# KdaiP/StableTTS

Measured on NVIDIA B200. Metric: mel-frames/sec through CFM DiT estimator (ODE solve, all evaluations), higher is better.
Workload: dtype f32 (split-bf16x3 tensor-core operands; FFN convs fp16 activations x fp16 hi/lo weights, 2 passes; fp32 accumulate)

## Files before the change

stabletts_b200/csrc/gemm_epilogue.cuh:

```cuda
#pragma once
#include "common.cuh"
#include <cstdlib>
#include "tc_ptx.cuh"

namespace st {

enum : int { EM_PLAIN = 0, EM_SILU = 1, EM_GELU = 2, EM_ROPE = 3, EM_LN = 4, EM_RESID = 5 };

struct EpiMaps { CUtensorMap o_f32, o_hi, o_lo, o2_f32, u_hi, u_lo, resid; };

struct TcParams {
    int n_src, Cs0, Cs1, taps, N, a_bmod, BB, T;
    int m_tiles_per_b, n_tiles, total_tiles;
    int flags, B, film_H, c_clamp, resid_clamp, rope_H, tap_outer;
    long film_bstride, gate_bstride;
    const float *bias, *mask, *film, *gate, *resid, *rope_cs;
    int mode;
    int has_f32, has_split;
    int out16, u16;
    int ln_mask_out, has_film2;
    const float *ln_shift, *ln_scale, *film2;
    long ada_bstride, film2_bstride;
    int ksplit, split_bb;
    long long* dbg;
// ... 12 lines not shown
    p.n_src = g.n_src; p.Cs0 = g.Cs[0]; p.Cs1 = g.Cs[1]; p.taps = g.taps; p.N = g.N; p.a_bmod = g.a_bmod; p.BB = g.BB; p.T = g.T;
    p.flags = g.flags; p.B = g.B; p.film_H = g.film_H; p.c_clamp = g.c_clamp; p.resid_clamp = g.resid_clamp; p.rope_H = g.rope_H;
    p.film_bstride = g.film_bstride; p.gate_bstride = g.gate_bstride;
    p.bias = g.bias; p.mask = g.mask; p.film = g.film; p.gate = g.gate; p.resid = g.resid; p.rope_cs = g.rope_cs;
    p.mode = epilogue_mode(g);
    p.has_f32 = g.out_f32 != nullptr; p.has_split = g.out_hi != nullptr;
    p.out16 = g.out16; p.u16 = g.u16;
    p.ln_mask_out = g.ln_mask_out; p.has_film2 = g.film2 != nullptr;
    p.ln_shift = g.ln_shift; p.ln_scale = g.ln_scale; p.film2 = g.film2;
    p.ada_bstride = g.ada_bstride; p.film2_bstride = g.film2_bstride;
    p.dbg = nullptr;
    p.ksplit = 1; p.split_bb = g.BB;
    static int tap_outer = -1;
    if (tap_outer < 0) { const char* e = getenv("STABLETTS_B200_TAP_OUTER"); tap_outer = (e && e[0] == '1') ? 1 : 0; }
    p.tap_outer = tap_outer;
}

constexpr float kQScale = 0.125f * 1.4426950408889634f;

constexpr int EPI_WARPS = 8;
constexpr int EPI_STAGE_BYTES = 4096;

namespace epi {

using namespace ptx;

__device__ __forceinline__ float4 ldg_keep(const float* p) {
    float4 v;
    asm volatile("ld.global.nc.L1::evict_last.v4.f32 {%0, %1, %2, %3}, [%4];" : "=f"(v.x), "=f"(v.y), "=f"(v.z), "=f"(v.w) : "l"(p));
    return v;
}
__device__ __forceinline__ float4 ldg_stream(const float* p) {
    float4 v;
    asm volatile("ld.global.nc.L1::no_allocate.v4.f32 {%0, %1, %2, %3}, [%4];" : "=f"(v.x), "=f"(v.y), "=f"(v.z), "=f"(v.w) : "l"(p));
    return v;
}
__device__ __forceinline__ void prefetch_l2(const float* p) { asm volatile("prefetch.global.L2 [%0];" ::"l"(p)); }

__device__ __forceinline__ float4 colvec(const float* v, int n, int N) { return ldg_keep(v + min(n, N - 4)); }

__device__ __forceinline__ void stage_f32(uint32_t stg, int lane, const float (&x)[32]) {
    const uint32_t row = stg + (uint32_t)lane * 128u;
#pragma unroll
    for (int q = 0; q < 8; ++q)
        st_shared_v4(row + (uint32_t)((q ^ (lane & 7)) << 4), __float_as_uint(x[4 * q]), __float_as_uint(x[4 * q + 1]),
                     __float_as_uint(x[4 * q + 2]), __float_as_uint(x[4 * q + 3]));
}

__device__ __forceinline__ void stage_split(uint32_t stg_hi, uint32_t stg_lo, int lane, const float (&x)[32]) {
    const uint32_t off = (uint32_t)lane * 64u;
    const uint32_t sw = (uint32_t)((lane >> 1) & 3);
#pragma unroll
    for (int c = 0; c < 4; ++c) {
        uint32_t h[4], l[4];
#pragma unroll
        for (int e = 0; e < 4; ++e) split_bf16x2(x[8 * c + 2 * e], x[8 * c + 2 * e + 1], h[e], l[e]);
        const uint32_t o = off + (((uint32_t)c ^ sw) << 4);
        st_shared_v4(stg_hi + o, h[0], h[1], h[2], h[3]);
        st_shared_v4(stg_lo + o, l[0], l[1], l[2], l[3]);
    }
}

__device__ __forceinline__ void stage_f16(uint32_t stg, int lane, const float (&x)[32]) {
    const uint32_t off = (uint32_t)lane * 64u;
    const uint32_t sw = (uint32_t)((lane >> 1) & 3);
#pragma unroll
    for (int c = 0; c < 4; ++c)
        st_shared_v4(stg + off + (((uint32_t)c ^ sw) << 4), pack_f16x2_sat(x[8 * c], x[8 * c + 1]), pack_f16x2_sat(x[8 * c + 2], x[8 * c + 3]),
                     pack_f16x2_sat(x[8 * c + 4], x[8 * c + 5]), pack_f16x2_sat(x[8 * c + 6], x[8 * c + 7]));
}

}

struct EpiCtx {
    int bb, t0, n0, mb, lane;
    uint32_t tacc, stg;
    float m, mrow;
    int tile_it;
    bool plain, has_resid, mask_only;
    const float *film, *gate, *resid_row;
    float s1, s2, kshift;
    uint32_t rbuf; uint64_t* rbar; uint32_t* rphase; int rb;
    int kstep;
};

template <bool ON>
__device__ __forceinline__ void epi_load_resid(const TcParams& p, const EpiCtx& c, float (&r)[32], int nb) {
    if constexpr (ON) {
#pragma unroll
        for (int q = 0; q < 8; ++q) {
            float4 v4 = make_float4(0.f, 0.f, 0.f, 0.f);
            if (c.has_resid) v4 = __ldg(reinterpret_cast<const float4*>(c.resid_row + min(nb + 4 * q, p.N - 4)));
            r[4 * q] = v4.x; r[4 * q + 1] = v4.y; r[4 * q + 2] = v4.z; r[4 * q + 3] = v4.w;
        }
    }
}

__device__ __forceinline__ void epi_resid_issue(const TcParams& p, const EpiMaps& em, const EpiCtx& c, int kc) {
    using namespace ptx;
    if (c.lane == 0) {
        uint64_t* bar = c.rbar + (kc & 1);
        mbar_expect_tx(bar, 4096);
        tma_load_3d_addr(&em.resid, bar, c.rbuf + (uint32_t)(kc & 1) * 4096u, c.n0 + kc * 32, c.t0, c.rb);
    }
}
__device__ __forceinline__ void epi_resid_take(EpiCtx& c, int kc, float (&r)[32]) {
    using namespace ptx;
    const int b = kc & 1;
    mbar_wait(c.rbar + b, (*c.rphase >> b) & 1u);
    *c.rphase ^= 1u << b;
    const uint32_t row = c.rbuf + (uint32_t)b * 4096u + (uint32_t)c.lane * 128u;
#pragma unroll
    for (int q = 0; q < 8; ++q) {
        float4 v4;
        asm volatile("ld.shared.v4.f32 {%0, %1, %2, %3}, [%4];" : "=f"(v4.x), "=f"(v4.y), "=f"(v4.z), "=f"(v4.w)
                     : "r"(row + (uint32_t)((q ^ (c.lane & 7)) << 4)));
        r[4 * q] = v4.x; r[4 * q + 1] = v4.y; r[4 * q + 2] = v4.z; r[4 * q + 3] = v4.w;
    }
    __syncwarp();
}

__device__ __forceinline__ void epi_store_f32(const CUtensorMap* map, const EpiCtx& c, int nb, const float (&x)[32]) {
    using namespace ptx;
    if (c.lane == 0) bulk_wait_read0();
    __syncwarp();
    epi::stage_f32(c.stg, c.lane, x);
    fence_proxy_async_smem();
    __syncwarp();
    if (c.lane == 0) { tma_store_3d(map, c.stg, nb, c.t0, c.bb); bulk_commit(); }
}
__device__ __forceinline__ void epi_store_split(const CUtensorMap* mhi, const CUtensorMap* mlo, const EpiCtx& c, int nb, const float (&x)[32]) {
    using namespace ptx;
    if (c.lane == 0) bulk_wait_read0();
    __syncwarp();
    epi::stage_split(c.stg, c.stg + 2048u, c.lane, x);
    fence_proxy_async_smem();
    __syncwarp();
    if (c.lane == 0) { tma_store_3d(mhi, c.stg, nb, c.t0, c.bb); tma_store_3d(mlo, c.stg + 2048u, nb, c.t0, c.bb); bulk_commit(); }
}

__device__ __forceinline__ void epi_store_f16(const CUtensorMap* map, const EpiCtx& c, int nb, const float (&x)[32]) {
    using namespace ptx;
    if (c.lane == 0) bulk_wait_read0();
    __syncwarp();
    epi::stage_f16(c.stg, c.lane, x);
    fence_proxy_async_smem();
    __syncwarp();
    if (c.lane == 0) { tma_store_3d(map, c.stg, nb, c.t0, c.bb); bulk_commit(); }
}

template <int BN, int MODE, bool TRES>
__device__ __forceinline__ void epi_chunk(const TcParams& p, const EpiMaps& em, EpiCtx& c, const float (&cs)[32], int kc,
                                          uint32_t (&v)[32], uint32_t (&vnext)[32], float (&r)[32]) {
    using namespace ptx;
    using namespace epi;
    constexpr int NCH = BN / 32;
    constexpr bool ROPE = MODE == EM_ROPE, LN = MODE == EM_LN, RES = MODE == EM_RESID || MODE == EM_LN;
    const int c0 = kc * 32, nb = c.n0 + c0;
    const bool trace = p.dbg != nullptr && blockIdx.x == 0 && threadIdx.x == 128 && c.tile_it < 8;
    long long tk0 = 0, tk1 = 0, tk2 = 0;
    if (trace) tk0 = clock64();
    float4 bq[8];
    if (nb < p.N && (p.flags & EPI_BIAS)) {
#pragma unroll
        for (int q = 0; q < 8; ++q) bq[q] = colvec(p.bias, nb + 4 * q, p.N);
    } else {
#pragma unroll
        for (int q = 0; q < 8; ++q) bq[q] = make_float4(0.f, 0.f, 0.f, 0.f);
    }
    tmem_ld_wait();
    const bool has_next = kc + c.kstep < NCH && nb + 32 * c.kstep < p.N;
    if (has_next) tmem_ld32(c.tacc + (uint32_t)(c0 + 32 * c.kstep), vnext);
    if (nb >= p.N) return;
    if constexpr (RES && TRES) {
        if (c.has_resid) {
            epi_resid_take(c, kc, r);
            if (kc + 2 < NCH && nb + 64 < p.N) epi_resid_issue(p, em, c, kc + 2);
        }
    }
    if (trace) tk1 = clock64();
    float x[32];
#pragma unroll
    for (int q = 0; q < 8; ++q) {
        x[4 * q] = __uint_as_float(v[4 * q]) + bq[q].x; x[4 * q + 1] = __uint_as_float(v[4 * q + 1]) + bq[q].y;
        x[4 * q + 2] = __uint_as_float(v[4 * q + 2]) + bq[q].z; x[4 * q + 3] = __uint_as_float(v[4 * q + 3]) + bq[q].w;
    }
    if constexpr (ROPE) {
        if (nb < 2 * p.rope_H && (nb & 63) == 0) {
#pragma unroll
            for (int j = 0; j < 16; ++j) {
                const float a = x[j], b = x[j + 16], co = cs[2 * j], si = cs[2 * j + 1];
                x[j] = a * co - b * si;
                x[j + 16] = b * co + a * si;
            }
        }
        if (nb < p.rope_H) {
#pragma unroll
            for (int j = 0; j < 32; ++j) x[j] *= kQScale;
        }
    } else {
        if constexpr (MODE == EM_SILU) {
#pragma unroll
            for (int j = 0; j < 32; ++j) x[j] = silu_fast(x[j]);
        }
        if constexpr (MODE == EM_GELU) {
#pragma unroll
            for (int j = 0; j < 32; ++j) x[j] = gelu_f(x[j]);
        }
        if (c.mask_only) {
#pragma unroll
            for (int j = 0; j < 32; ++j) x[j] *= c.m;
        } else if (!c.plain) {
            if (p.flags & EPI_FILM) {
                float4 fg[8], fb[8];
#pragma unroll
                for (int q = 0; q < 8; ++q) { fg[q] = colvec(c.film, nb + 4 * q, p.N); fb[q] = colvec(c.film + p.film_H, nb + 4 * q, p.N); }
#pragma unroll
                for (int q = 0; q < 8; ++q) {
                    x[4 * q] = fmaf(fg[q].x, x[4 * q], fb[q].x); x[4 * q + 1] = fmaf(fg[q].y, x[4 * q + 1], fb[q].y);
                    x[4 * q + 2] = fmaf(fg[q].z, x[4 * q + 2], fb[q].z); x[4 * q + 3] = fmaf(fg[q].w, x[4 * q + 3], fb[q].w);
                }
            }
            float4 g4[8];
            if (p.flags & EPI_GATE) {
#pragma unroll
                for (int q = 0; q < 8; ++q) g4[q] = colvec(c.gate, nb + 4 * q, p.N);
#pragma unroll
                for (int q = 0; q < 8; ++q) { g4[q].x *= c.m; g4[q].y *= c.m; g4[q].z *= c.m; g4[q].w *= c.m; }
            } else {
#pragma unroll
                for (int q = 0; q < 8; ++q) g4[q] = make_float4(c.m, c.m, c.m, c.m);
            }
#pragma unroll
            for (int q = 0; q < 8; ++q) {
                if constexpr (RES) {
                    x[4 * q] = fmaf(x[4 * q], g4[q].x, r[4 * q]); x[4 * q + 1] = fmaf(x[4 * q + 1], g4[q].y, r[4 * q + 1]);
                    x[4 * q + 2] = fmaf(x[4 * q + 2], g4[q].z, r[4 * q + 2]); x[4 * q + 3] = fmaf(x[4 * q + 3], g4[q].w, r[4 * q + 3]);
                } else {
                    x[4 * q] *= g4[q].x; x[4 * q + 1] *= g4[q].y; x[4 * q + 2] *= g4[q].z; x[4 * q + 3] *= g4[q].w;
                }
            }
        }
        if constexpr (!TRES) { if (has_next) epi_load_resid<RES>(p, c, r, nb + 32 * c.kstep); }
    }
    if (trace) tk2 = clock64();
    if (p.has_f32) epi_store_f32(&em.o_f32, c, nb, x);
    if (p.has_split) { if (p.out16) epi_store_f16(&em.o_hi, c, nb, x); else epi_store_split(&em.o_hi, &em.o_lo, c, nb, x); }
    if (trace) {
        long long* d = p.dbg + ((long)(c.tile_it >> 1) * 2 * NCH + kc) * 8;
        d[0] = tk0; d[1] = tk1; d[2] = tk2; d[3] = 0; d[4] = clock64();
    }
    if constexpr (LN) {
        if (p.has_film2) {
            const float* f2 = p.film2 + (long)c.mb * p.film2_bstride;
#pragma unroll
            for (int q = 0; q < 8; ++q) {
                const float4 fg = colvec(f2, nb + 4 * q, p.N), fb = colvec(f2 + p.film_H, nb + 4 * q, p.N);
                x[4 * q] = (fg.x * x[4 * q] + fb.x) * c.mrow; x[4 * q + 1] = (fg.y * x[4 * q + 1] + fb.y) * c.mrow;
                x[4 * q + 2] = (fg.z * x[4 * q + 2] + fb.z) * c.mrow; x[4 * q + 3] = (fg.w * x[4 * q + 3] + fb.w) * c.mrow;
            }
            epi_store_f32(&em.o2_f32, c, nb, x);
        }
        if (kc == 0) c.kshift = x[0];
        float a1 = 0.f, a2 = 0.f, b1 = 0.f, b2 = 0.f;
#pragma unroll
        for (int j = 0; j < 32; j += 2) {
            const float d0 = x[j] - c.kshift, d1 = x[j + 1] - c.kshift;
            a1 += d0; a2 = fmaf(d0, d0, a2); b1 += d1; b2 = fmaf(d1, d1, b2);
        }
        c.s1 += a1 + b1; c.s2 += a2 + b2;
#pragma unroll
        for (int j = 0; j < 32; ++j) v[j] = __float_as_uint(x[j]);
        tmem_st32(c.tacc + (uint32_t)c0, v);
        if (trace) p.dbg[((long)(c.tile_it >> 1) * 2 * NCH + kc) * 8 + 3] = clock64();
    }
}

template <int BN>
__device__ __forceinline__ void epi_chunk_ln2(const TcParams& p, const EpiMaps& em, const EpiCtx& c, float mean, float rstd, float mo,
                                              const float* sh, const float* sc, int kc, uint32_t (&v)[32], uint32_t (&vnext)[32]) {
    using namespace ptx;
    using namespace epi;
    constexpr int NCH = BN / 32;
    const int c0 = kc * 32, nb = c.n0 + c0;
    const bool trace = p.dbg != nullptr && blockIdx.x == 0 && threadIdx.x == 128 && c.tile_it < 8;
    long long tk0 = 0, tk1 = 0, tk2 = 0;
    if (trace) tk0 = clock64();
    tmem_ld_wait();
    if (kc + 1 < NCH) tmem_ld32(c.tacc + (uint32_t)(c0 + 32), vnext);
    if (trace) tk1 = clock64();
    float u[32];
#pragma unroll
    for (int q = 0; q < 8; ++q) {
        const float4 s4 = colvec(sh, nb + 4 * q, p.N), c4 = colvec(sc, nb + 4 * q, p.N);
        u[4 * q] = ((__uint_as_float(v[4 * q]) - mean) * rstd * (1.f + c4.x) + s4.x) * mo;
        u[4 * q + 1] = ((__uint_as_float(v[4 * q + 1]) - mean) * rstd * (1.f + c4.y) + s4.y) * mo;
        u[4 * q + 2] = ((__uint_as_float(v[4 * q + 2]) - mean) * rstd * (1.f + c4.z) + s4.z) * mo;
        u[4 * q + 3] = ((__uint_as_float(v[4 * q + 3]) - mean) * rstd * (1.f + c4.w) + s4.w) * mo;
    }
    if (trace) tk2 = clock64();
    if (p.u16) epi_store_f16(&em.u_hi, c, nb, u); else epi_store_split(&em.u_hi, &em.u_lo, c, nb, u);
    if (trace) {
        long long* d = p.dbg + ((long)(c.tile_it >> 1) * 2 * NCH + NCH + kc) * 8;
        d[0] = tk0; d[1] = tk1; d[2] = tk2; d[3] = 0; d[4] = clock64();
    }
}

struct ResidPipe { uint32_t buf = 0; uint64_t* bar = nullptr; uint32_t phase = 0; };

template <int BN, int MODE, bool TRES, class WaitFn>
__device__ __forceinline__ void epilogue_tile(const TcParams& p, const EpiMaps& em, int bb, int t0, int n0, uint32_t tacc,
                                              uint32_t stg, int lane, int tile_it, ResidPipe& rp, int split_group,
                                              WaitFn wait_accumulator) {
    using namespace ptx;
    using namespace epi;
    constexpr int NCH = BN / 32;
    constexpr bool ROPE = MODE == EM_ROPE, LN = MODE == EM_LN, RES = MODE == EM_RESID || MODE == EM_LN;
    const int tcl = min(t0 + lane, p.T - 1);
    EpiCtx c;
    c.bb = bb; c.t0 = t0; c.n0 = n0; c.mb = bb % p.B; c.lane = lane;
    c.tacc = tacc; c.stg = stg;
    c.tile_it = tile_it;
    c.plain = ROPE || (p.flags & (EPI_FILM | EPI_MASK | EPI_GATE | EPI_RESID)) == 0;
    c.mask_only = !ROPE && (p.flags & (EPI_FILM | EPI_MASK | EPI_GATE | EPI_RESID)) == EPI_MASK;
    c.has_resid = RES && (p.flags & EPI_RESID);
    c.m = 1.f; c.mrow = 1.f; c.film = nullptr; c.gate = nullptr; c.resid_row = nullptr;
    c.s1 = 0.f; c.s2 = 0.f; c.kshift = 0.f;
    c.rbuf = rp.buf; c.rbar = rp.bar; c.rphase = &rp.phase; c.rb = min(bb, p.resid_clamp);
    const int k0 = split_group >= 0 ? split_group : 0;
    c.kstep = split_group >= 0 ? 2 : 1;
    float cs[32];
    float ra[32];
    if constexpr (ROPE) {
        const float4* q = reinterpret_cast<const float4*>(p.rope_cs + (long)tcl * 32);
#pragma unroll
        for (int i = 0; i < 8; ++i) {
            const float4 c4 = __ldg(q + i);
            cs[4 * i] = c4.x; cs[4 * i + 1] = c4.y; cs[4 * i + 2] = c4.z; cs[4 * i + 3] = c4.w;
        }
    } else {
        if (p.mask) c.mrow = __ldg(p.mask + (long)c.mb * p.T + tcl);
        if (p.flags & EPI_MASK) c.m = c.mrow;
        c.film = p.film + (long)c.mb * p.film_bstride;
        c.gate = p.gate + (long)min(bb, p.c_clamp) * p.gate_bstride;
        c.resid_row = p.resid + ((long)min(bb, p.resid_clamp) * p.T + tcl) * p.N;
        if constexpr (RES && TRES) {
            if (c.has_resid) {
                epi_resid_issue(p, em, c, 0);
                if (NCH > 1 && n0 + 32 < p.N) epi_resid_issue(p, em, c, 1);
            }
        } else {
            epi_load_resid<RES>(p, c, ra, n0 + 32 * k0);
        }
    }

    const bool trace_tile = p.dbg != nullptr && blockIdx.x == 0 && threadIdx.x == 128 && tile_it < 8;
    long long tt0 = 0, tt1 = 0;
    if (trace_tile) tt0 = clock64();
    wait_accumulator();
    if (trace_tile) tt1 = clock64();

    uint32_t va[32], vb[32];
    tmem_ld32(tacc + (uint32_t)(32 * k0), va);
#pragma unroll 1
    for (int kc = k0; kc < NCH; kc += 2 * c.kstep) {
        epi_chunk<BN, MODE, TRES>(p, em, c, cs, kc, va, vb, ra);
        epi_chunk<BN, MODE, TRES>(p, em, c, cs, kc + c.kstep, vb, va, ra);
    }

    if constexpr (LN) {
        tmem_st_wait();
        const float inv_n = 1.0f / (float)p.N;
        const float dm = c.s1 * inv_n;
        const float mean = c.kshift + dm;
        const float rstd = rsqrtf(fmaxf(c.s2 * inv_n - dm * dm, 0.f) + 1e-5f);
        const float mo = p.ln_mask_out ? c.mrow : 1.0f;
        const float* sh = p.ln_shift + (long)min(bb, p.c_clamp) * p.ada_bstride;
        const float* sc = p.ln_scale + (long)min(bb, p.c_clamp) * p.ada_bstride;
        tmem_ld32(tacc, va);
#pragma unroll 1
        for (int kc = 0; kc < NCH; kc += 2) {
            epi_chunk_ln2<BN>(p, em, c, mean, rstd, mo, sh, sc, kc, va, vb);
            epi_chunk_ln2<BN>(p, em, c, mean, rstd, mo, sh, sc, kc + 1, vb, va);
        }
    }
    if (trace_tile) {
        long long* d = p.dbg + ((long)(tile_it >> 1) * 2 * NCH) * 8;
        d[5] = tt0; d[6] = tt1; d[7] = clock64();
    }
}

}
```

stabletts_b200/csrc/gemm_tc.cu:

```cuda
#include "common.cuh"
#include "gemm_epilogue.cuh"
#include <cuda.h>
#include <cudaTypedefs.h>
#include <mutex>
#include <unordered_map>
#include <string>
#include <cstring>
#include <cstdlib>

namespace st {

bool build_epi_maps(const GemmArgs& g, EpiMaps* em);
bool tmap_encode_bf16(const void* ptr, int rank, uint64_t d0, uint64_t d1, uint64_t d2, uint32_t b0, uint32_t b1,
                      CUtensorMap* out);

namespace {

constexpr int BLOCK_M = 128;
constexpr int BLOCK_K = 64;
constexpr int UMMA_K = 16;
constexpr int NUM_THREADS = 384;
constexpr int A_TILE_BYTES = BLOCK_M * BLOCK_K * 2;

struct TcMaps {
// ... 52 lines not shown
    pdl_wait();

    if (warp == 0) {
        if (elect_one()) {
            int stage = 0; uint32_t phase = 0;
            for (int tile = blockIdx.x; tile < p.total_tiles; tile += gridDim.x) {
                const int n_tile = tile % p.n_tiles, m_tile = tile / p.n_tiles;
                const int bb = m_tile / p.m_tiles_per_b, t0 = (m_tile % p.m_tiles_per_b) * BLOCK_M;
                const int ab = (bb % p.split_bb) % p.a_bmod, n0 = n_tile * BN;
                const int it_per = (num_kb + p.ksplit - 1) / p.ksplit;
                const int it0 = (bb / p.split_bb) * it_per, it1 = min(num_kb, it0 + it_per);
                for (int it = it0; it < it1; ++it) {
                    {
                        const int kb = p.tap_outer ? it % kb_per_tap : it / p.taps;
                        const int tap = p.tap_outer ? it / kb_per_tap : it % p.taps;
                        const int src = kb >= kb0 ? 1 : 0;
                        const int kc = (src ? kb - kb0 : kb) * BLOCK_K;
                        const int kw = (src ? p.Cs0 : 0) + kc;
                        mbar_wait(&empty_bar[stage], phase ^ 1);
                        uint8_t* s = smem + stage * C::STAGE_BYTES;
                        mbar_expect_tx(&full_bar[stage], C::STAGE_BYTES);
                        tma_load_3d(&maps.a_hi[src], &full_bar[stage], s, kc, t0 + tap - pad, ab);
                        tma_load_3d(&maps.a_lo[src], &full_bar[stage], s + A_TILE_BYTES, kc, t0 + tap - pad, ab);
                        tma_load_2d(&maps.w_hi, &full_bar[stage], s + 2 * A_TILE_BYTES, kw, tap * p.N + n0);
                        tma_load_2d(&maps.w_lo, &full_bar[stage], s + 2 * A_TILE_BYTES + C::B_TILE_BYTES, kw, tap * p.N + n0);
                        if (++stage == C::STAGES) { stage = 0; phase ^= 1; }
                    }
                }
            }
        }
    } else if (warp == 1) {
        constexpr uint32_t idesc = make_idesc_bf16(BLOCK_M, BN);
        int stage = 0; uint32_t phase = 0;
        int acc = 0; uint32_t acc_phase = 0;
        for (int tile = blockIdx.x; tile < p.total_tiles; tile += gridDim.x) {
            mbar_wait(&tmem_empty[acc], acc_phase ^ 1);
            tc_fence_after();
            const uint32_t tmem_d = tmem_base + acc * BN;
            int n_it = num_kb;
            if (p.ksplit > 1) {
                const int bb = (tile / p.n_tiles) / p.m_tiles_per_b;
                const int it_per = (num_kb + p.ksplit - 1) / p.ksplit;
                const int it0 = (bb / p.split_bb) * it_per;
                n_it = min(num_kb, it0 + it_per) - it0;
            }
            for (int kb = 0; kb < n_it; ++kb) {
                mbar_wait(&full_bar[stage], phase);
                tc_fence_after();
                if (elect_one()) {
                    const uint32_t sa = smem_u32(smem + stage * C::STAGE_BYTES);
                    const uint64_t a_hi = make_sw128_desc(sa), a_lo = make_sw128_desc(sa + A_TILE_BYTES);
                    const uint64_t b_hi = make_sw128_desc(sa + 2 * A_TILE_BYTES);
                    const uint64_t b_lo = make_sw128_desc(sa + 2 * A_TILE_BYTES + C::B_TILE_BYTES);
#pragma unroll
                    for (int k = 0; k < BLOCK_K / UMMA_K; ++k) {
                        const uint64_t adv = (uint64_t)((k * UMMA_K * 2) >> 4);
                        umma_bf16(tmem_d, a_lo + adv, b_hi + adv, idesc, (kb | k) != 0);
                        umma_bf16(tmem_d, a_hi + adv, b_lo + adv, idesc, 1);
                        umma_bf16(tmem_d, a_hi + adv, b_hi + adv, idesc, 1);
                    }
                    umma_commit(&empty_bar[stage]);
                    if (kb == n_it - 1) umma_commit(&tmem_full[acc]);
                }
                __syncwarp();
                if (++stage == C::STAGES) { stage = 0; phase ^= 1; }
            }
            if (++acc == 2) { acc = 0; acc_phase ^= 1; }
        }
    } else if (warp >= 4) {
        const int wq = warp & 3, grp = (warp - 4) >> 2;
        const uint32_t stg = smem_u32(smem + C::STAGING_OFF + (warp - 4) * EPI_STAGE_BYTES);
        if (lane == 0) {
            prefetch_tmap(&em.o_f32); prefetch_tmap(&em.o_hi); prefetch_tmap(&em.o_lo);
        }
        const bool split = p.total_tiles <= (int)gridDim.x;
        const int acc = split ? 0 : grp;
        ResidPipe rp;
        int tile_it = split ? 0 : grp; uint32_t acc_phase = 0;
        for (int tile = blockIdx.x + (split ? 0 : grp * gridDim.x); tile < p.total_tiles; tile += 2 * gridDim.x, tile_it += 2) {
            const int n_tile = tile % p.n_tiles, m_tile = tile / p.n_tiles;
            const int bb = m_tile / p.m_tiles_per_b, t0 = (m_tile % p.m_tiles_per_b) * BLOCK_M + wq * 32;
            const uint32_t tacc = tmem_base + ((uint32_t)(wq * 32) << 16) + (uint32_t)(acc * BN);
            uint64_t* fb = &tmem_full[acc];
            const uint32_t ph = acc_phase;
            epilogue_tile<BN, MODE, false>(p, em, bb, t0, n_tile * BN, tacc, stg, lane, tile_it, rp, split ? grp : -1, [fb, ph]() { mbar_wait(fb, ph); tc_fence_after(); });
            tc_fence_before();
            __syncwarp();
            if (lane == 0) mbar_arrive(&tmem_empty[acc]);
            acc_phase ^= 1;
        }
        if (lane == 0) bulk_wait_read0();
    }

    tc_fence_before();
    __syncthreads();
    if (warp == 2) {
        tc_fence_after();
        asm volatile("tcgen05.dealloc.cta_group::1.sync.aligned.b32 %0, %1;" ::"r"(tmem_base), "n"(C::TMEM_COLS));
    }
}

std::string g_err = "";
std::mutex g_mu;
PFN_cuTensorMapEncodeTiled_v12000 g_encode = nullptr;

struct MapKey {
    const void* ptr; uint64_t d0, d1, d2; uint32_t b0, b1; int rank;
    bool operator==(const MapKey& o) const {
        return ptr == o.ptr && d0 == o.d0 && d1 == o.d1 && d2 == o.d2 && b0 == o.b0 && b1 == o.b1 && rank == o.rank;
    }
};
struct MapKeyHash {
    size_t operator()(const MapKey& k) const {
        size_t h = std::hash<const void*>()(k.ptr);
        h ^= k.d0 * 0x9E3779B97F4A7C15ull + (h << 6); h ^= k.d1 * 0xC2B2AE3D27D4EB4Full + (h >> 3);
        h ^= k.d2 * 0x165667B19E3779F9ull + (h << 9); h ^= ((size_t)k.b0 << 20) ^ ((size_t)k.b1 << 4) ^ (size_t)k.rank;
        return h;
    }
};
std::unordered_map<MapKey, CUtensorMap, MapKeyHash> g_maps;

bool ensure_encode() {
    if (g_encode) return true;
    void* fn = nullptr;
    cudaDriverEntryPointQueryResult qres;
    cudaError_t e = cudaGetDriverEntryPoint("cuTensorMapEncodeTiled", &fn, cudaEnableDefault, &qres);
    if (e != cudaSuccess || qres != cudaDriverEntryPointSuccess || !fn) {
        g_err = "cuTensorMapEncodeTiled driver entry point unavailable";
        return false;
    }
    g_encode = reinterpret_cast<PFN_cuTensorMapEncodeTiled_v12000>(fn);
    return true;
}

bool get_map(const void* ptr, int rank, uint64_t d0, uint64_t d1, uint64_t d2, uint32_t b0, uint32_t b1, CUtensorMap* out,
             int kind = 0) {
    MapKey key{ptr, d0, d1, d2, b0, b1, rank | (kind << 8)};
    auto it = g_maps.find(key);
    if (it != g_maps.end()) { *out = it->second; return true; }
    const uint64_t es = kind == 1 ? 4 : 2;
    cuuint64_t dims[3] = {d0, d1, d2};
    cuuint64_t strides[2] = {d0 * es, d0 * d1 * es};
    cuuint32_t box[3] = {b0, b1, 1};
    cuuint32_t estr[3] = {1, 1, 1};
    CUtensorMap m;
    CUresult r = g_encode(&m, kind == 1 ? CU_TENSOR_MAP_DATA_TYPE_FLOAT32 : CU_TENSOR_MAP_DATA_TYPE_BFLOAT16, (cuuint32_t)rank,
                          const_cast<void*>(ptr), dims, strides, box, estr, CU_TENSOR_MAP_INTERLEAVE_NONE,
                          kind == 2 ? CU_TENSOR_MAP_SWIZZLE_64B : CU_TENSOR_MAP_SWIZZLE_128B,
                          kind == 0 ? CU_TENSOR_MAP_L2_PROMOTION_L2_256B : CU_TENSOR_MAP_L2_PROMOTION_NONE,
                          CU_TENSOR_MAP_FLOAT_OOB_FILL_NONE);
    if (r != CUDA_SUCCESS) {
        g_err = "cuTensorMapEncodeTiled failed with CUresult " + std::to_string((int)r) + " (rank " + std::to_string(rank) +
                ", dims " + std::to_string(d0) + "x" + std::to_string(d1) + "x" + std::to_string(d2) + ")";
        return false;
    }
    if (g_maps.size() > 4096) g_maps.clear();
    g_maps.emplace(key, m);
    *out = m;
    return true;
}

template <int BN, int MODE>
cudaError_t launch_inst(const TcMaps& maps, const EpiMaps& em, const TcParams& p, int grid, cudaStream_t s) {
    using C = Cfg<BN>;
    static std::atomic<uint64_t> attr_done{0};
    cudaError_t e = ensure_dyn_smem(gemm_tc_kernel<BN, MODE>, C::SMEM_BYTES, attr_done);
    if (e != cudaSuccess) { g_err = "cudaFuncSetAttribute(max dynamic smem) failed"; return e; }
    return launch_k(gemm_tc_kernel<BN, MODE>, dim3(grid), dim3(NUM_THREADS), (size_t)C::SMEM_BYTES, s, maps, em, p);
}

template <int BN>
// ... 152 lines not shown
```

stabletts_b200/csrc/gemm_tc2.cu:

```cuda
#include "common.cuh"
#include "tc_ptx.cuh"
#include "gemm_epilogue.cuh"
#include <string>
#include <cstdlib>
#include <cstring>

namespace st {

bool tmap_encode_bf16(const void* ptr, int rank, uint64_t d0, uint64_t d1, uint64_t d2, uint32_t b0, uint32_t b1,
                      CUtensorMap* out);
bool build_epi_maps(const GemmArgs& g, EpiMaps* em);
const char* gemm_tc_last_error();

namespace {

using namespace ptx;

constexpr int BM = 128;
constexpr int BK = 64;
constexpr int UK = 16;
constexpr int THREADS = 384;
constexpr int TILE_BYTES = 128 * BK * 2;

template <int BN2, int SHALLOW = 0, int PREC = 0> struct Cfg2 {
    static constexpr int B_TILE_BYTES = (BN2 / 2) * BK * 2;
    static constexpr int A_PLANES = PREC ? 1 : 2;
    static constexpr int STAGE_BYTES = A_PLANES * TILE_BYTES + 2 * B_TILE_BYTES;
    static constexpr int STAGES = SHALLOW ? 2 : (PREC ? 4 : (BN2 == 256 ? 3 : 4));
    static constexpr int TMEM_COLS = 2 * BN2;
    static constexpr int STAGING_OFF = STAGES * STAGE_BYTES;
    static constexpr int RESID_OFF = STAGING_OFF + EPI_WARPS * EPI_STAGE_BYTES;
    static constexpr int BAR_OFF = RESID_OFF + (SHALLOW ? EPI_WARPS * 2 * 4096 : 0);
    static constexpr int SMEM_BYTES = BAR_OFF + 256 + 1024;
};

struct Maps2 { CUtensorMap a_hi[2], a_lo[2], w_hi, w_lo; };

typedef TcParams Params2;

template <int BN2, int MODE, int SHALLOW, int PREC>
__global__ void __cluster_dims__(2, 1, 1) __launch_bounds__(THREADS, 1)
gemm_tc2_kernel(const __grid_constant__ Maps2 maps, const __grid_constant__ EpiMaps em, const Params2 p) {
    using CF = Cfg2<BN2, SHALLOW, PREC>;
    constexpr int A_BYTES = CF::A_PLANES * TILE_BYTES;
    constexpr int B_TILE_BYTES = CF::B_TILE_BYTES, STAGE_BYTES = CF::STAGE_BYTES, STAGES = CF::STAGES;
    constexpr int TMEM_COLS = CF::TMEM_COLS;
    extern __shared__ uint8_t smem_raw[];
    uint8_t* smem = reinterpret_cast<uint8_t*>((reinterpret_cast<uintptr_t>(smem_raw) + 1023) & ~uintptr_t(1023));
    uint64_t* full_bar = reinterpret_cast<uint64_t*>(smem + CF::BAR_OFF);
    uint64_t* empty_bar = full_bar + STAGES;
    uint64_t* tmem_full = empty_bar + STAGES;
    uint64_t* tmem_empty = tmem_full + 2;
    uint64_t* resid_bar = tmem_empty + 2;
    uint32_t* tmem_slot = reinterpret_cast<uint32_t*>(resid_bar + 2 * EPI_WARPS);

    pdl_trigger();
    const int warp = threadIdx.x >> 5, lane = threadIdx.x & 31;
    const uint32_t rank = cluster_ctarank();
    const bool leader = rank == 0;
    const int cluster_id = blockIdx.x >> 1, num_clusters = gridDim.x >> 1;
    const int kb0 = (p.Cs0 + BK - 1) / BK;
    const int kb1 = p.n_src > 1 ? (p.Cs1 + BK - 1) / BK : 0;
    const int kb_per_tap = kb0 + kb1;
    const int num_kb = p.taps * kb_per_tap;
    const int pad = p.taps / 2;

    if (warp == 0 && lane == 0) {
        prefetch_tmap(&maps.a_hi[0]); prefetch_tmap(&maps.a_lo[0]); prefetch_tmap(&maps.w_hi); prefetch_tmap(&maps.w_lo);
        if (p.n_src > 1) { prefetch_tmap(&maps.a_hi[1]); prefetch_tmap(&maps.a_lo[1]); }
    }
    if (warp == 1 && lane == 0) {
        for (int i = 0; i < STAGES; ++i) { mbar_init(&full_bar[i], 1); mbar_init(&empty_bar[i], 1); }
        for (int i = 0; i < 2; ++i) { mbar_init(&tmem_full[i], 1); mbar_init(&tmem_empty[i], EPI_WARPS); }
        if (SHALLOW) for (int i = 0; i < 2 * EPI_WARPS; ++i) mbar_init(&resid_bar[i], 1);
        mbar_fence_init();
    }
    if (warp == 2) tmem_alloc_2sm<TMEM_COLS>(tmem_slot);
    tc_fence_before();
    cluster_sync();
    tc_fence_after();
    const uint32_t tmem_base = *tmem_slot;
    pdl_wait();

    if (warp == 0) {
        if (elect_one()) {
            int stage = 0; uint32_t phase = 0;
            for (int tile = cluster_id; tile < p.total_tiles; tile += num_clusters) {
                const int n_tile = tile % p.n_tiles, m_tile = tile / p.n_tiles;
                const int bb = m_tile / p.m_tiles_per_b, t0 = (m_tile % p.m_tiles_per_b) * (2 * BM) + (int)rank * BM;
                const int ab = bb % p.a_bmod, n0 = n_tile * BN2 + (int)rank * (BN2 / 2);
                for (int it = 0; it < num_kb; ++it) {
                    {
                        const int kb = p.tap_outer ? it % kb_per_tap : it / p.taps;
                        const int tap = p.tap_outer ? it / kb_per_tap : it % p.taps;
                        const int src = kb >= kb0 ? 1 : 0;
                        const int kc = (src ? kb - kb0 : kb) * BK;
                        const int kw = (src ? p.Cs0 : 0) + kc;
                        mbar_wait(&empty_bar[stage], phase ^ 1);
                        uint8_t* s = smem + stage * STAGE_BYTES;
                        if (leader) mbar_expect_tx(&full_bar[stage], 2 * STAGE_BYTES);
                        tma_load_3d_2sm(&maps.a_hi[src], &full_bar[stage], s, kc, t0 + tap - pad, ab);
                        if (!PREC) tma_load_3d_2sm(&maps.a_lo[src], &full_bar[stage], s + TILE_BYTES, kc, t0 + tap - pad, ab);
                        tma_load_2d_2sm(&maps.w_hi, &full_bar[stage], s + A_BYTES, kw, tap * p.N + n0);
                        tma_load_2d_2sm(&maps.w_lo, &full_bar[stage], s + A_BYTES + B_TILE_BYTES, kw, tap * p.N + n0);
                        if (++stage == STAGES) { stage = 0; phase ^= 1; }
                    }
                }
            }
        }
    } else if (warp == 1) {
        if (leader) {
            constexpr uint32_t idesc = PREC ? make_idesc_f16(2 * BM, BN2) : make_idesc_bf16(2 * BM, BN2);
            int stage = 0; uint32_t phase = 0;
            int acc = 0; uint32_t acc_phase = 0;
            for (int tile = cluster_id; tile < p.total_tiles; tile += num_clusters) {
                mbar_wait(&tmem_empty[acc], acc_phase ^ 1);
                tc_fence_after();
                const uint32_t tmem_d = tmem_base + acc * BN2;
                for (int kb = 0; kb < num_kb; ++kb) {
                    mbar_wait(&full_bar[stage], phase);
                    tc_fence_after();
                    if (elect_one()) {
                        const uint32_t sa = smem_u32(smem + stage * STAGE_BYTES);
                        const uint64_t a_hi = make_sw128_desc(sa), a_lo = make_sw128_desc(sa + TILE_BYTES);
                        const uint64_t b_hi = make_sw128_desc(sa + A_BYTES), b_lo = make_sw128_desc(sa + A_BYTES + B_TILE_BYTES);
#pragma unroll
                        for (int k = 0; k < BK / UK; ++k) {
                            const uint64_t adv = (uint64_t)((k * UK * 2) >> 4);
                            if (PREC) {
                                umma_bf16_2sm(tmem_d, a_hi + adv, b_lo + adv, idesc, (kb | k) != 0);
                                umma_bf16_2sm(tmem_d, a_hi + adv, b_hi + adv, idesc, 1);
                            } else {
                                umma_bf16_2sm(tmem_d, a_lo + adv, b_hi + adv, idesc, (kb | k) != 0);
                                umma_bf16_2sm(tmem_d, a_hi + adv, b_lo + adv, idesc, 1);
                                umma_bf16_2sm(tmem_d, a_hi + adv, b_hi + adv, idesc, 1);
                            }
                        }
                        umma_commit_2sm(&empty_bar[stage], 0b11);
                        if (kb == num_kb - 1) umma_commit_2sm(&tmem_full[acc], 0b11);
                    }
                    __syncwarp();
                    if (++stage == STAGES) { stage = 0; phase ^= 1; }
                }
                if (++acc == 2) { acc = 0; acc_phase ^= 1; }
            }
        }
    } else if (warp >= 4) {
        const int wq = warp & 3, grp = (warp - 4) >> 2;
        const uint32_t stg = smem_u32(smem + CF::STAGING_OFF + (warp - 4) * EPI_STAGE_BYTES);
        if (lane == 0) {
            prefetch_tmap(&em.o_f32); prefetch_tmap(&em.o_hi); prefetch_tmap(&em.o_lo);
            if (MODE == EM_LN) { prefetch_tmap(&em.u_hi); prefetch_tmap(&em.u_lo); prefetch_tmap(&em.o2_f32); }
            if (SHALLOW) prefetch_tmap(&em.resid);
        }
        ResidPipe rp;
        if (SHALLOW) { rp.buf = smem_u32(smem + CF::RESID_OFF + (warp - 4) * 2 * 4096); rp.bar = resid_bar + 2 * (warp - 4); }
        const bool split = MODE != EM_LN && !SHALLOW && p.total_tiles <= num_clusters;
        const int acc = split ? 0 : grp;
        int tile_it = split ? 0 : grp; uint32_t acc_phase = 0;
        for (int tile = cluster_id + (split ? 0 : grp * num_clusters); tile < p.total_tiles; tile += 2 * num_clusters, tile_it += 2) {
            const int n_tile = tile % p.n_tiles, m_tile = tile / p.n_tiles;
            const int bb = m_tile / p.m_tiles_per_b;
            const int t0 = (m_tile % p.m_tiles_per_b) * (2 * BM) + (int)rank * BM + wq * 32;
            const uint32_t tacc = tmem_base + ((uint32_t)(wq * 32) << 16) + (uint32_t)(acc * BN2);
            uint64_t* fb = &tmem_full[acc];
            const uint32_t ph = acc_phase;
            epilogue_tile<BN2, MODE, SHALLOW != 0>(p, em, bb, t0, n_tile * BN2, tacc, stg, lane, tile_it, rp, split ? grp : -1, [fb, ph]() { mbar_wait(fb, ph); tc_fence_after(); });
            tc_fence_before();
            __syncwarp();
            if (lane == 0) mbar_arrive_cluster(&tmem_empty[acc], 0);
            acc_phase ^= 1;
        }
        if (lane == 0) bulk_wait_read0();
    }

    tc_fence_before();
    cluster_sync();
    if (warp == 2) {
        tc_fence_after();
        tmem_dealloc_2sm<TMEM_COLS>(tmem_base);
    }
}

std::string g_err2;
long long* g_epi_trace = nullptr;

}

int gemm_tc2_read_trace(long long* host_out) {
    if (!g_epi_trace) return 1;
    return cudaMemcpy(host_out, g_epi_trace, 4 * 16 * 8 * sizeof(long long), cudaMemcpyDeviceToHost) == cudaSuccess ? 0 : 1;
}

const char* gemm_tc2_last_error() { return g_err2.c_str(); }

bool gemm_tc2_eligible(const GemmArgs& g, int num_sms) {
    if (g.N < 256 || g.N % 128) return false;
    const long pair_tiles = (long)g.BB * ((g.T + 255) / 256) * ((g.N + 255) / 256);
    return pair_tiles >= (num_sms / 2);
}

static int pick_bn2(const GemmArgs& g, int pairs) {
    static int forced = -1;
    if (forced < 0) { const char* e = getenv("STABLETTS_B200_TC2_BN"); forced = e ? atoi(e) : 0; }
    if (g.ln) return 256;
    if (forced == 128 || forced == 256) return forced;
    const long m_tiles = (long)g.BB * ((g.T + 2 * BM - 1) / (2 * BM));
    const long t256 = m_tiles * ((g.N + 255) / 256), t128 = m_tiles * ((g.N + 127) / 128);
    const double w256 = (double)((t256 + pairs - 1) / pairs), w128 = 0.515 * (double)((t128 + pairs - 1) / pairs);
    return w128 < 0.97 * w256 ? 128 : 256;
}

template <int BN2, int MODE, int SHALLOW, int PREC = 0>
static cudaError_t launch_tc2_inst(const Maps2& maps, const EpiMaps& em, const Params2& p, int pairs, cudaStream_t s) {
    static std::atomic<uint64_t> attr_done{0};
    using CF = Cfg2<BN2, SHALLOW, PREC>;
    cudaError_t e = ensure_dyn_smem(gemm_tc2_kernel<BN2, MODE, SHALLOW, PREC>, CF::SMEM_BYTES, attr_done);
    if (e != cudaSuccess) { g_err2 = "cudaFuncSetAttribute(max dynamic smem) failed for gemm_tc2_kernel"; return e; }
    const int clusters = p.total_tiles < pairs ? p.total_tiles : pairs;
    return launch_k(gemm_tc2_kernel<BN2, MODE, SHALLOW, PREC>, dim3(2 * clusters), dim3(THREADS), (size_t)CF::SMEM_BYTES, s, maps, em, p);
}

static bool use_shallow(const GemmArgs& g) {
    static int env = -1;
    if (env < 0) { const char* e = getenv("STABLETTS_B200_SHALLOW"); env = (e && !strcmp(e, "0")) ? 0 : 1; }
    return env && (g.flags & EPI_RESID) && g.resid && (long)g.Ktot * g.taps <= 512;
}

template <int BN2>
static cudaError_t launch_tc2_bn(const Maps2& maps, const EpiMaps& em, Params2& p, const GemmArgs& g, int pairs, cudaStream_t s) {
    p.n_tiles = (g.N + BN2 - 1) / BN2;
    p.total_tiles = g.BB * p.m_tiles_per_b * p.n_tiles;
    const bool sh = use_shallow(g);
    if (g.prec) {
        switch (p.mode) {
            case EM_SILU:  return launch_tc2_inst<BN2, EM_SILU, 0, 1>(maps, em, p, pairs, s);
            case EM_LN:    return launch_tc2_inst<BN2, EM_LN, 0, 1>(maps, em, p, pairs, s);
            case EM_RESID: return launch_tc2_inst<BN2, EM_RESID, 0, 1>(maps, em, p, pairs, s);
            case EM_PLAIN: return launch_tc2_inst<BN2, EM_PLAIN, 0, 1>(maps, em, p, pairs, s);
            default: g_err2 = "the two-pass fp16 precision is built for the FFN and long-skip convs only"; return cudaErrorInvalidValue;
        }
    }
    switch (p.mode) {
        case EM_ROPE: return launch_tc2_inst<BN2, EM_ROPE, 0>(maps, em, p, pairs, s);
        case EM_LN:   return sh ? launch_tc2_inst<BN2, EM_LN, 1>(maps, em, p, pairs, s) : launch_tc2_inst<BN2, EM_LN, 0>(maps, em, p, pairs, s);
        case EM_SILU: return launch_tc2_inst<BN2, EM_SILU, 0>(maps, em, p, pairs, s);
        case EM_GELU: return launch_tc2_inst<BN2, EM_GELU, 0>(maps, em, p, pairs, s);
        case EM_RESID: return sh ? launch_tc2_inst<BN2, EM_RESID, 1>(maps, em, p, pairs, s) : launch_tc2_inst<BN2, EM_RESID, 0>(maps, em, p, pairs, s);
        default:      return launch_tc2_inst<BN2, EM_PLAIN, 0>(maps, em, p, pairs, s);
    }
}

cudaError_t launch_gemm_tc2(const GemmArgs& g, int num_sms, cudaStream_t s) {
    Maps2 maps;
// ... 32 lines not shown
```

Baseline: 609,100.

## Release TMEM accumulators early and use more accumulator buffers in 2-SM GEMM

Epilogue warps now signal the tmem_empty barrier as soon as the last TMEM chunk has been loaded into registers, instead of after the whole tile's stores. The MMA warp can therefore start the next tile sooner. The 2-SM kernel also sizes its accumulator ring as 512/BN2 buffers, up to four for smaller BN2, instead of a fixed two, so the MMA can run further ahead of the epilogue. This adds more complex phase and index bookkeeping, and the LN path has to release only after its second pass.

```diff
diff --git a/stabletts_b200/csrc/gemm_epilogue.cuh b/stabletts_b200/csrc/gemm_epilogue.cuh
--- a/stabletts_b200/csrc/gemm_epilogue.cuh
+++ b/stabletts_b200/csrc/gemm_epilogue.cuh
@@ -118,6 +118,7 @@
     float s1, s2, kshift;
     uint32_t rbuf; uint64_t* rbar; uint32_t* rphase; int rb;
     int kstep;
+    bool released;
 };
 
 template <bool ON>
@@ -185,9 +186,14 @@
     if (c.lane == 0) { tma_store_3d(map, c.stg, nb, c.t0, c.bb); bulk_commit(); }
 }
 
-template <int BN, int MODE, bool TRES>
+template <class ReleaseFn>
+__device__ __forceinline__ void epi_release(EpiCtx& c, ReleaseFn release) {
+    if (!c.released) { ptx::tc_fence_before(); __syncwarp(); release(); c.released = true; }
+}
+
+template <int BN, int MODE, bool TRES, class ReleaseFn>
 __device__ __forceinline__ void epi_chunk(const TcParams& p, const EpiMaps& em, EpiCtx& c, const float (&cs)[32], int kc,
-                                          uint32_t (&v)[32], uint32_t (&vnext)[32], float (&r)[32]) {
+                                          uint32_t (&v)[32], uint32_t (&vnext)[32], float (&r)[32], ReleaseFn release) {
     using namespace ptx;
     using namespace epi;
     constexpr int NCH = BN / 32;
@@ -207,6 +213,7 @@
     tmem_ld_wait();
     const bool has_next = kc + c.kstep < NCH && nb + 32 * c.kstep < p.N;
     if (has_next) tmem_ld32(c.tacc + (uint32_t)(c0 + 32 * c.kstep), vnext);
+    else if constexpr (!LN) epi_release(c, release);
     if (nb >= p.N) return;
     if constexpr (RES && TRES) {
         if (c.has_resid) {
@@ -312,9 +319,10 @@
     }
 }
 
-template <int BN>
-__device__ __forceinline__ void epi_chunk_ln2(const TcParams& p, const EpiMaps& em, const EpiCtx& c, float mean, float rstd, float mo,
-                                              const float* sh, const float* sc, int kc, uint32_t (&v)[32], uint32_t (&vnext)[32]) {
+template <int BN, class ReleaseFn>
+__device__ __forceinline__ void epi_chunk_ln2(const TcParams& p, const EpiMaps& em, EpiCtx& c, float mean, float rstd, float mo,
+                                              const float* sh, const float* sc, int kc, uint32_t (&v)[32], uint32_t (&vnext)[32],
+                                              ReleaseFn release) {
     using namespace ptx;
     using namespace epi;
     constexpr int NCH = BN / 32;
@@ -324,6 +332,7 @@
     if (trace) tk0 = clock64();
     tmem_ld_wait();
     if (kc + 1 < NCH) tmem_ld32(c.tacc + (uint32_t)(c0 + 32), vnext);
+    else epi_release(c, release);
     if (trace) tk1 = clock64();
     float u[32];
 #pragma unroll
@@ -344,10 +353,10 @@
 
 struct ResidPipe { uint32_t buf = 0; uint64_t* bar = nullptr; uint32_t phase = 0; };
 
-template <int BN, int MODE, bool TRES, class WaitFn>
+template <int BN, int MODE, bool TRES, class WaitFn, class ReleaseFn>
 __device__ __forceinline__ void epilogue_tile(const TcParams& p, const EpiMaps& em, int bb, int t0, int n0, uint32_t tacc,
                                               uint32_t stg, int lane, int tile_it, ResidPipe& rp, int split_group,
-                                              WaitFn wait_accumulator) {
+                                              WaitFn wait_accumulator, ReleaseFn release) {
     using namespace ptx;
     using namespace epi;
     constexpr int NCH = BN / 32;
@@ -365,6 +374,7 @@
     c.rbuf = rp.buf; c.rbar = rp.bar; c.rphase = &rp.phase; c.rb = min(bb, p.resid_clamp);
     const int k0 = split_group >= 0 ? split_group : 0;
     c.kstep = split_group >= 0 ? 2 : 1;
+    c.released = false;
     float cs[32];
     float ra[32];
     if constexpr (ROPE) {
@@ -400,8 +410,8 @@
     tmem_ld32(tacc + (uint32_t)(32 * k0), va);
 #pragma unroll 1
     for (int kc = k0; kc < NCH; kc += 2 * c.kstep) {
-        epi_chunk<BN, MODE, TRES>(p, em, c, cs, kc, va, vb, ra);
-        epi_chunk<BN, MODE, TRES>(p, em, c, cs, kc + c.kstep, vb, va, ra);
+        epi_chunk<BN, MODE, TRES>(p, em, c, cs, kc, va, vb, ra, release);
+        epi_chunk<BN, MODE, TRES>(p, em, c, cs, kc + c.kstep, vb, va, ra, release);
     }
 
     if constexpr (LN) {
@@ -416,8 +426,8 @@
         tmem_ld32(tacc, va);
 #pragma unroll 1
         for (int kc = 0; kc < NCH; kc += 2) {
-            epi_chunk_ln2<BN>(p, em, c, mean, rstd, mo, sh, sc, kc, va, vb);
-            epi_chunk_ln2<BN>(p, em, c, mean, rstd, mo, sh, sc, kc + 1, vb, va);
+            epi_chunk_ln2<BN>(p, em, c, mean, rstd, mo, sh, sc, kc, va, vb, release);
+            epi_chunk_ln2<BN>(p, em, c, mean, rstd, mo, sh, sc, kc + 1, vb, va, release);
         }
     }
     if (trace_tile) {
diff --git a/stabletts_b200/csrc/gemm_tc.cu b/stabletts_b200/csrc/gemm_tc.cu
--- a/stabletts_b200/csrc/gemm_tc.cu
+++ b/stabletts_b200/csrc/gemm_tc.cu
@@ -158,11 +158,11 @@
             const int bb = m_tile / p.m_tiles_per_b, t0 = (m_tile % p.m_tiles_per_b) * BLOCK_M + wq * 32;
             const uint32_t tacc = tmem_base + ((uint32_t)(wq * 32) << 16) + (uint32_t)(acc * BN);
             uint64_t* fb = &tmem_full[acc];
+            uint64_t* eb = &tmem_empty[acc];
             const uint32_t ph = acc_phase;
-            epilogue_tile<BN, MODE, false>(p, em, bb, t0, n_tile * BN, tacc, stg, lane, tile_it, rp, split ? grp : -1, [fb, ph]() { mbar_wait(fb, ph); tc_fence_after(); });
-            tc_fence_before();
-            __syncwarp();
-            if (lane == 0) mbar_arrive(&tmem_empty[acc]);
+            epilogue_tile<BN, MODE, false>(p, em, bb, t0, n_tile * BN, tacc, stg, lane, tile_it, rp, split ? grp : -1,
+                                           [fb, ph]() { mbar_wait(fb, ph); tc_fence_after(); },
+                                           [eb, lane]() { if (lane == 0) mbar_arrive(eb); });
             acc_phase ^= 1;
         }
         if (lane == 0) bulk_wait_read0();
diff --git a/stabletts_b200/csrc/gemm_tc2.cu b/stabletts_b200/csrc/gemm_tc2.cu
--- a/stabletts_b200/csrc/gemm_tc2.cu
+++ b/stabletts_b200/csrc/gemm_tc2.cu
@@ -27,11 +27,13 @@
     static constexpr int A_PLANES = PREC ? 1 : 2;
     static constexpr int STAGE_BYTES = A_PLANES * TILE_BYTES + 2 * B_TILE_BYTES;
     static constexpr int STAGES = SHALLOW ? 2 : (PREC ? 4 : (BN2 == 256 ? 3 : 4));
-    static constexpr int TMEM_COLS = 2 * BN2;
+    static constexpr int ACC = 512 / BN2;
+    static constexpr int TMEM_COLS = ACC * BN2;
     static constexpr int STAGING_OFF = STAGES * STAGE_BYTES;
     static constexpr int RESID_OFF = STAGING_OFF + EPI_WARPS * EPI_STAGE_BYTES;
     static constexpr int BAR_OFF = RESID_OFF + (SHALLOW ? EPI_WARPS * 2 * 4096 : 0);
-    static constexpr int SMEM_BYTES = BAR_OFF + 256 + 1024;
+    static constexpr int SMEM_BYTES = BAR_OFF + 512 + 1024;
+    static_assert(SMEM_BYTES <= 227 * 1024, "dynamic shared memory above the per-block limit");
 };
 
 struct Maps2 { CUtensorMap a_hi[2], a_lo[2], w_hi, w_lo; };
@@ -44,14 +46,14 @@
     using CF = Cfg2<BN2, SHALLOW, PREC>;
     constexpr int A_BYTES = CF::A_PLANES * TILE_BYTES;
     constexpr int B_TILE_BYTES = CF::B_TILE_BYTES, STAGE_BYTES = CF::STAGE_BYTES, STAGES = CF::STAGES;
-    constexpr int TMEM_COLS = CF::TMEM_COLS;
+    constexpr int TMEM_COLS = CF::TMEM_COLS, ACC = CF::ACC;
     extern __shared__ uint8_t smem_raw[];
     uint8_t* smem = reinterpret_cast<uint8_t*>((reinterpret_cast<uintptr_t>(smem_raw) + 1023) & ~uintptr_t(1023));
     uint64_t* full_bar = reinterpret_cast<uint64_t*>(smem + CF::BAR_OFF);
     uint64_t* empty_bar = full_bar + STAGES;
     uint64_t* tmem_full = empty_bar + STAGES;
-    uint64_t* tmem_empty = tmem_full + 2;
-    uint64_t* resid_bar = tmem_empty + 2;
+    uint64_t* tmem_empty = tmem_full + ACC;
+    uint64_t* resid_bar = tmem_empty + ACC;
     uint32_t* tmem_slot = reinterpret_cast<uint32_t*>(resid_bar + 2 * EPI_WARPS);
 
     pdl_trigger();
@@ -71,7 +73,7 @@
     }
     if (warp == 1 && lane == 0) {
         for (int i = 0; i < STAGES; ++i) { mbar_init(&full_bar[i], 1); mbar_init(&empty_bar[i], 1); }
-        for (int i = 0; i < 2; ++i) { mbar_init(&tmem_full[i], 1); mbar_init(&tmem_empty[i], EPI_WARPS); }
+        for (int i = 0; i < ACC; ++i) { mbar_init(&tmem_full[i], 1); mbar_init(&tmem_empty[i], EPI_WARPS); }
         if (SHALLOW) for (int i = 0; i < 2 * EPI_WARPS; ++i) mbar_init(&resid_bar[i], 1);
         mbar_fence_init();
     }
@@ -142,7 +144,7 @@
                     __syncwarp();
                     if (++stage == STAGES) { stage = 0; phase ^= 1; }
                 }
-                if (++acc == 2) { acc = 0; acc_phase ^= 1; }
+                if (++acc == ACC) { acc = 0; acc_phase ^= 1; }
             }
         }
     } else if (warp >= 4) {
@@ -156,20 +158,19 @@
         ResidPipe rp;
         if (SHALLOW) { rp.buf = smem_u32(smem + CF::RESID_OFF + (warp - 4) * 2 * 4096); rp.bar = resid_bar + 2 * (warp - 4); }
         const bool split = MODE != EM_LN && !SHALLOW && p.total_tiles <= num_clusters;
-        const int acc = split ? 0 : grp;
-        int tile_it = split ? 0 : grp; uint32_t acc_phase = 0;
-        for (int tile = cluster_id + (split ? 0 : grp * num_clusters); tile < p.total_tiles; tile += 2 * num_clusters, tile_it += 2) {
+        int tile_it = split ? 0 : grp, acc = split ? 0 : grp; uint32_t acc_phase = 0;
+        for (int tile = cluster_id + (split ? 0 : grp * num_clusters); tile < p.total_tiles;
+             tile += 2 * num_clusters, tile_it += 2, acc += 2) {
+            if (acc >= ACC) { acc -= ACC; acc_phase ^= 1; }
             const int n_tile = tile % p.n_tiles, m_tile = tile / p.n_tiles;
             const int bb = m_tile / p.m_tiles_per_b;
             const int t0 = (m_tile % p.m_tiles_per_b) * (2 * BM) + (int)rank * BM + wq * 32;
             const uint32_t tacc = tmem_base + ((uint32_t)(wq * 32) << 16) + (uint32_t)(acc * BN2);
             uint64_t* fb = &tmem_full[acc];
-            const uint32_t ph = acc_phase;
-            epilogue_tile<BN2, MODE, SHALLOW != 0>(p, em, bb, t0, n_tile * BN2, tacc, stg, lane, tile_it, rp, split ? grp : -1, [fb, ph]() { mbar_wait(fb, ph); tc_fence_after(); });
-            tc_fence_before();
-            __syncwarp();
-            if (lane == 0) mbar_arrive_cluster(&tmem_empty[acc], 0);
-            acc_phase ^= 1;
+            uint64_t* eb = &tmem_empty[acc];
+            epilogue_tile<BN2, MODE, SHALLOW != 0>(p, em, bb, t0, n_tile * BN2, tacc, stg, lane, tile_it, rp, split ? grp : -1,
+                                                   [fb, acc_phase]() { mbar_wait(fb, acc_phase); tc_fence_after(); },
+                                                   [eb, lane]() { if (lane == 0) mbar_arrive_cluster(eb, 0); });
         }
         if (lane == 0) bulk_wait_read0();
     }
```

Result: no change. 613,800 (median of 6 runs) (+0.8%).
